# qzwlecr/p1

Measured on AMD Instinct MI355X. Metric: SHA-256 nonce-hashes/sec (GH/s), higher is better.
Workload: dtype u32

## Files before the change

### p1_amd/__init__.py

```python
from ._lib import (
    P1HipError,
    lib_path,
    load,
    init,
    init_devices,
    scan,
    scan_batch,
    batch_layout,
    get_batch_stats,
    hash,
    reduce_pairs,
    plan_shards,
    set_profiling,
    get_stats,
    get_device_stats,
    reset_stats,
    device_count,
    device_info,
    comm_info,
    abi_version,
    ABI_VERSION,
    test_knobs,
    shutdown,
    version,
    codeobj_bytes,
    codeobj_sha256,
    batch_codeobj_sha256,
)
from .sharding import shard_range, combine_keys
```

### p1_amd/_lib.py

```python
import ctypes
import os

_HERE = os.path.dirname(os.path.abspath(__file__))
_LIB = None

U64 = ctypes.c_uint64


class P1HipError(RuntimeError):
    def __init__(self, rc, msg):
        super().__init__(f"p1hip rc={rc}: {msg}")
        self.rc = rc


class Stats(ctypes.Structure):
    _fields_ = [
        ("scans", U64),
        ("fast_launches", U64),
        ("fast_nonces", U64),
        ("fast_alg_ops", U64),
        ("generic_launches", U64),
        ("generic_nonces", U64),
        ("scan_wall_ms", ctypes.c_double),
        ("scan_launches", U64),
# ... 45 lines not shown
        ("launches", U64),
        ("tiles", U64),
        ("nonces", U64),
        ("wall_ms", ctypes.c_double),
    ]

    def as_dict(self):
        return {k: getattr(self, k) for k, _ in self._fields_}


class DeviceInfo(ctypes.Structure):
    _fields_ = [
        ("ordinal", ctypes.c_int32),
        ("cu_count", ctypes.c_int32),
        ("clock_khz", ctypes.c_int32),
        ("reserved", ctypes.c_int32),
        ("hbm_bytes", U64),
        ("pci_bus_id", ctypes.c_char * 32),
        ("arch", ctypes.c_char * 32),
        ("uuid", ctypes.c_ubyte * 16),
    ]

    def as_dict(self):
        return {"ordinal": self.ordinal, "cu_count": self.cu_count, "clock_khz": self.clock_khz,
                "hbm_bytes": self.hbm_bytes, "pci_bus_id": self.pci_bus_id.decode(errors="replace"),
                "arch": self.arch.decode(errors="replace"), "uuid": bytes(self.uuid).hex()}


def lib_path():
    return os.environ.get("P1HIP_LIB") or os.path.join(_HERE, "libp1hip.so")


SIGNATURES = [
    ("p1hip_init", ctypes.c_int, [ctypes.c_int, ctypes.POINTER(ctypes.c_int)]),
    ("p1hip_init_devices", ctypes.c_int, [ctypes.POINTER(ctypes.c_int), ctypes.c_int]),
    ("p1hip_scan", ctypes.c_int,
     [ctypes.c_char_p, ctypes.c_size_t, U64, U64, ctypes.POINTER(U64), ctypes.POINTER(U64)]),
    ("p1hip_scan_batch", ctypes.c_int, [ctypes.POINTER(Request), ctypes.c_size_t, ctypes.POINTER(Result)]),
    ("p1hip_batch_layout", ctypes.c_int,
     [ctypes.POINTER(Request), ctypes.c_size_t, ctypes.c_int, ctypes.POINTER(ctypes.c_uint32),
      ctypes.POINTER(ctypes.c_int32), ctypes.POINTER(ctypes.c_int32)]),
    ("p1hip_get_batch_stats", ctypes.c_int, [ctypes.POINTER(BatchStats)]),
    ("p1hip_hash", ctypes.c_int, [ctypes.c_char_p, ctypes.c_size_t, U64, ctypes.POINTER(U64)]),
    ("p1hip_plan_shards", ctypes.c_int,
     [ctypes.c_char_p, ctypes.c_size_t, U64, U64, ctypes.c_int, ctypes.POINTER(U64), ctypes.POINTER(U64)]),
    ("p1hip_reduce_pairs", ctypes.c_int,
     [ctypes.POINTER(U64), ctypes.POINTER(U64), ctypes.c_size_t, ctypes.POINTER(U64), ctypes.POINTER(U64)]),
    ("p1hip_set_profiling", ctypes.c_int, [ctypes.c_int]),
    ("p1hip_get_stats", ctypes.c_int, [ctypes.POINTER(Stats)]),
    ("p1hip_reset_stats", None, []),
    ("p1hip_get_device_stats", ctypes.c_int, [ctypes.c_int, ctypes.POINTER(DeviceStats)]),
    ("p1hip_device_count", ctypes.c_int, []),
    ("p1hip_device_info", ctypes.c_int, [ctypes.c_int, ctypes.POINTER(DeviceInfo)]),
    ("p1hip_comm_info", ctypes.c_int, [ctypes.c_int, ctypes.POINTER(ctypes.c_int), ctypes.POINTER(ctypes.c_int)]),
    ("p1hip_abi_version", ctypes.c_int, []),
    ("p1hip_test_knobs", ctypes.c_char_p, []),
    ("p1hip_last_error", ctypes.c_char_p, []),
    ("p1hip_version", ctypes.c_char_p, []),
    ("p1hip_shutdown", None, []),
]


def load(path=None):
    global _LIB
    if _LIB is not None and path is None:
        return _LIB
    p = path or lib_path()
    if not os.path.exists(p):
        raise P1HipError(-100, f"{p} not built (run `make` or __graft_entry__.build())")
    lib = ctypes.CDLL(p)
    for name, res, args in SIGNATURES:
        fn = getattr(lib, name)
        fn.restype = res
        fn.argtypes = args
    if lib.p1hip_abi_version() != ABI_VERSION:
        raise P1HipError(-100, f"{p}: ABI version {lib.p1hip_abi_version()}, this binding reads version "
                               f"{ABI_VERSION} structs (rebuild the library)")
    if path is None:
        _LIB = lib
    return lib


def _check(rc):
    if rc != 0:
        raise P1HipError(rc, load().p1hip_last_error().decode(errors="replace"))


def _bytes(msg):
    if isinstance(msg, str):
        return msg.encode("utf-8")
    return bytes(msg)


def init(want_devices=0):
    got = ctypes.c_int(0)
    _check(load().p1hip_init(int(want_devices), ctypes.byref(got)))
    return got.value


def init_devices(ordinals):
    arr = (ctypes.c_int * len(ordinals))(*ordinals)
    _check(load().p1hip_init_devices(arr, len(ordinals)))


def scan(msg, lower, upper):
    m = _bytes(msg)
    h, n = U64(), U64()
    _check(load().p1hip_scan(m, len(m), int(lower), int(upper), ctypes.byref(h), ctypes.byref(n)))
    return h.value, n.value


def _requests(requests):
    rows = [(_bytes(m), int(lo), int(hi)) for m, lo, hi in requests]
    arr = (Request * max(len(rows), 1))()
    for r, (m, lo, hi) in zip(arr, rows):
        r.msg, r.msg_len, r.lower, r.upper = m, len(m), lo, hi
    return arr, rows


def scan_batch(requests):
    arr, rows = _requests(requests)
    out = (Result * max(len(rows), 1))()
    _check(load().p1hip_scan_batch(arr, len(rows), out))
    return [(out[i].hash, out[i].nonce) for i in range(len(rows))]


def batch_layout(requests, ndev):
    arr, rows = _requests(requests)
    n = len(rows)
    tiles = (ctypes.c_uint32 * max(n, 1))()
    device = (ctypes.c_int32 * max(n, 1))()
    launch = (ctypes.c_int32 * max(n, 1))()
    _check(load().p1hip_batch_layout(arr, n, int(ndev), tiles, device, launch))
    return [{"tiles": tiles[i], "device": device[i], "launch": launch[i]} for i in range(n)]


def get_batch_stats():
    s = BatchStats()
    _check(load().p1hip_get_batch_stats(ctypes.byref(s)))
    return s.as_dict()


def batch_codeobj_sha256(lib=None):
    import hashlib

    lib = lib or load()
    start = ctypes.addressof(ctypes.c_char.in_dll(lib, "p1hip_batch_co"))
    end = ctypes.addressof(ctypes.c_char.in_dll(lib, "p1hip_batch_co_end"))
    if end <= start:
        raise P1HipError(-100, "embedded batch code object is empty")
    return hashlib.sha256(ctypes.string_at(start, end - start)).hexdigest()


def hash(msg, nonce):
    m = _bytes(msg)
    h = U64()
    _check(load().p1hip_hash(m, len(m), int(nonce), ctypes.byref(h)))
    return h.value


def plan_shards(msg, lower, upper, n):
    m = _bytes(msg)
    first, last = (U64 * n)(), (U64 * n)()
    _check(load().p1hip_plan_shards(m, len(m), int(lower), int(upper), int(n), first, last))
    return [(a, b) if a <= b else None for a, b in zip(first, last)]


def reduce_pairs(hashes, nonces):
    n = len(hashes)
    assert n == len(nonces)
    ha = (U64 * max(n, 1))(*hashes)
    na = (U64 * max(n, 1))(*nonces)
    h, o = U64(), U64()
    _check(load().p1hip_reduce_pairs(ha, na, n, ctypes.byref(h), ctypes.byref(o)))
    return h.value, o.value


def set_profiling(on):
    _check(load().p1hip_set_profiling(1 if on else 0))


def get_stats():
    s = Stats()
    _check(load().p1hip_get_stats(ctypes.byref(s)))
    return s.as_dict()


def get_device_stats(index):
    s = DeviceStats()
    _check(load().p1hip_get_device_stats(int(index), ctypes.byref(s)))
    return s.as_dict()


def device_info(index):
    s = DeviceInfo()
    _check(load().p1hip_device_info(int(index), ctypes.byref(s)))
    return s.as_dict()


def comm_info(index):
    n, r = ctypes.c_int(0), ctypes.c_int(-1)
    _check(load().p1hip_comm_info(int(index), ctypes.byref(n), ctypes.byref(r)))
    return n.value, r.value


ABI_VERSION = 6


def abi_version():
    return load().p1hip_abi_version()


def test_knobs():
    raw = load().p1hip_test_knobs().decode()
    return dict(kv.split("=", 1) if "=" in kv else (kv, "?") for kv in raw.split(";") if kv)


def reset_stats():
    load().p1hip_reset_stats()


def device_count():
    return load().p1hip_device_count()


def shutdown():
    load().p1hip_shutdown()


def version():
    return load().p1hip_version().decode()


def codeobj_bytes(lib=None):
    lib = lib or load()
    start = ctypes.addressof(ctypes.c_char.in_dll(lib, "p1hip_kernels_co"))
    end = ctypes.addressof(ctypes.c_char.in_dll(lib, "p1hip_kernels_co_end"))
    if end <= start:
        raise P1HipError(-100, "embedded code object is empty")
    return ctypes.string_at(start, end - start)


def codeobj_sha256(lib=None):
    import hashlib

    return hashlib.sha256(codeobj_bytes(lib)).hexdigest()
```

### p1_amd/csrc/p1hip.hip

```cpp
#include <hip/hip_runtime.h>
#include <rccl/rccl.h>

#include <stdlib.h>
#include <string.h>

#include <algorithm>
#include <atomic>
#include <chrono>
#include <exception>
#include <mutex>
#include <string>
#include <thread>
#include <utility>
#include <vector>

#include "../../include/p1hip.h"
#include "batch_plan.hpp"
#include "planner.hpp"
#include "scan_abi.hpp"
#include "scan_pack.hpp"

extern "C" const unsigned char p1hip_kernels_co[];
extern "C" const unsigned char p1hip_batch_co[];

using namespace p1;

namespace {

thread_local std::string g_err;

int fail(int rc, const std::string& what) {
  g_err = what;
  return rc;
}

template <typename Fn>
int guarded(Fn&& fn) {
  try {
    return fn();
  } catch (const std::exception& ex) {
    return fail(P1HIP_ERR_HIP, std::string("host: ") + ex.what());
  } catch (...) {
    return fail(P1HIP_ERR_HIP, "host: unknown exception");
  }
}

#define HIPCHK(expr)                                                                        \
  do {                                                                                      \
    hipError_t e_ = (expr);                                                                 \
    if (e_ != hipSuccess)                                                                   \
      return fail(P1HIP_ERR_HIP, std::string(#expr) + ": " + hipGetErrorString(e_));       \
  } while (0)

#define NCCLCHK(expr)                                                                       \
  do {                                                                                      \
    ncclResult_t r_ = (expr);                                                               \
    if (r_ != ncclSuccess)                                                                  \
      return fail(P1HIP_ERR_RCCL, std::string(#expr) + ": " + ncclGetErrorString(r_));      \
  } while (0)

constexpr size_t kMaxKwTabs = 8;
constexpr uint64_t kMaxKwTabBytes = 8ull << 30;
constexpr uint64_t kMaxScanSpan = 1ull << 40;

enum KnobKind { kValue, kZeroDef, kFlag };
enum KnobWhen { kPerScan, kPerBatch, kAtInit };
enum KnobId {
  kSmallMaxNoncesKnob, kMaxLaunchBlocksKnob, kMaxScanSpanKnob, kKwtabMaxBytesKnob, kNoRcclKnob, kForceRcclKnob,
  kMinFastThreadsKnob, kTestFailDeviceKnob, kNoTableKnob, kNoSplitKnob, kScanGridKnob, kBatchMaxNoncesKnob,
  kBatchMaxTilesKnob, kKnobCount
};
struct Knob {
  const char* name;
  uint64_t def, max;
  KnobKind kind;
  KnobWhen when;
  const char* what;
};
const Knob kKnobs[] = {
    {"P1HIP_SMALL_MAX_NONCES", kSmallMaxNonces, kSmallMaxNonces, kValue, kPerScan,
     "shares of at most this many nonces take the one-launch small path; 0 turns it off, so small parity ranges "
     "run the fast kernel variants"},
    {"P1HIP_MAX_LAUNCH_BLOCKS", kMaxLaunchBlocks, kMaxLaunchBlocks, kZeroDef, kPerScan,
     "workgroups per k_scan launch, so GPU tests run the multi-launch path on small ranges; a larger piece gets "
     "a launch of its own (at most kMaxFastThreads / kBlock = 2^18 workgroups, far below HIP's grid limit)"},
    {"P1HIP_MAX_SCAN_SPAN", kMaxScanSpan, ~0ull, kZeroDef, kPerScan, "nonces per piece of a device's share"},
    {"P1HIP_KWTAB_MAX_BYTES", kMaxKwTabBytes, ~0ull, kValue, kPerScan,
     "MODE 5 table cap; a larger table re-plans the share without MODE 5"},
    {"P1HIP_NO_RCCL", 0, 1, kFlag, kAtInit,
     "combine the per-device results through the host, so the multi-device path (threads, sharding, combine) "
     "runs with the same GPU listed twice on a 1-GPU box"},
    {"P1HIP_FORCE_RCCL", 0, 1, kFlag, kAtInit, "a communicator even for one device"},
    {"P1HIP_MIN_FAST_THREADS", kMinFastThreads, ~0ull, kValue, kAtInit,
     "planner occupancy floor; 1 keeps k = 3 on small ranges so every k = 3 variant runs on the GPU"},
    {"P1HIP_TEST_FAIL_DEVICE", ~0ull, ~0ull, kValue, kAtInit,
     "device index whose scan phase reports a failure (the multi-device error path); default -1: none"},
    {"P1HIP_NO_TABLE", 0, 1, kFlag, kAtInit,
     "no MODE 5: layouts whose tail block 1 holds only lo digits run the digit-update variants (A/B, and a "
     "second kernel path to cross-check MODE 5)"},
    {"P1HIP_NO_SPLIT", 0, 1, kFlag, kAtInit,
     "straddling lo digits use mode 2 instead of the split modes (A/B builds with -DP1_NV2_PLAIN)"},
    {"P1HIP_SCAN_GRID", 0, kMaxLaunchBlocks, kZeroDef, kPerScan,
     "k_scan's grid instead of the device's workgroup slots (the default, 0); at or above a launch's tile count "
     "every workgroup runs one tile and the queue hands out none (the round-5 dispatch, same code object)"},
    {"P1HIP_BATCH_MAX_NONCES", kBatchMaxNonces, kBatchMaxNonces, kValue, kPerBatch,
     "requests of at most this many nonces are coalesced by p1hip_scan_batch; 0 runs every request "
     "individually; independent of P1HIP_SMALL_MAX_NONCES"},
    {"P1HIP_BATCH_MAX_TILES", kBatchMaxTiles, kBatchMaxTiles, kZeroDef, kPerBatch,
     "tiles per launch pair, so GPU tests run several launch pairs on small batches (batch_layout raises it to "
     "the largest single request's tile count)"},
};
static_assert(sizeof kKnobs / sizeof kKnobs[0] == kKnobCount, "one row per KnobId, in its order");

bool test_knobs_on() {
  const char* m = getenv("P1HIP_TEST_KNOBS");
  return m && m[0] == '1' && m[1] == 0;
}

const char* test_knob(const char* name) {
  if (!test_knobs_on()) return nullptr;
  const char* v = getenv(name);
  return v && *v ? v : nullptr;
}

uint64_t knob(KnobId id) {
  const Knob& K = kKnobs[id];
  const char* v = test_knob(K.name);
  if (!v) return K.def;
  if (K.kind == kFlag) return v[0] == '1';
  const uint64_t n = strtoull(v, nullptr, 10);
  if (n == 0 && K.kind == kZeroDef) return K.def;
  return n < K.max ? n : K.max;
}

template <typename T, bool kPinned>
struct Buf {
  T* p = nullptr;
  size_t cap = 0;

  Buf() = default;
  Buf(const Buf&) = delete;
  Buf(Buf&& o) noexcept : p(std::exchange(o.p, nullptr)), cap(std::exchange(o.cap, 0)) {}
  Buf& operator=(Buf&& o) noexcept {
    if (this != &o) {
      (void)release();
      p = std::exchange(o.p, nullptr);
      cap = std::exchange(o.cap, 0);
    }
    return *this;
  }
  ~Buf() { (void)release(); }

  hipError_t release() {
    hipError_t e = hipSuccess;
    if (p) e = kPinned ? hipHostFree(p) : hipFree(p);
    p = nullptr;
    cap = 0;
    return e;
  }
  hipError_t reserve(size_t need, size_t floor, size_t extra = 0) {
    if (need <= cap) return hipSuccess;
    hipError_t e = release();
    if (e != hipSuccess) return e;
    size_t n = floor;
    while (n < need) n <<= 1;
    const size_t bytes = (n + extra) * sizeof(T);
    e = kPinned ? hipHostMalloc(&p, bytes, hipHostMallocDefault) : hipMalloc(&p, bytes);
    if (e != hipSuccess) p = nullptr;
    else cap = n;
    return e;
  }
};
template <typename T> using DevBuf = Buf<T, false>;
template <typename T> using PinnedBuf = Buf<T, true>;

struct Dev {
  int ordinal = -1;
  hipStream_t stream = nullptr;
  DevBuf<Key> d_part;
  DevBuf<Key> d_res;
  DevBuf<Key> d_gather;
  PinnedBuf<Key> h_res;
  DevBuf<Segment> d_seg;
  PinnedBuf<Segment> h_seg;
  ncclComm_t comm = nullptr;
  hipModule_t mod = nullptr;
  hipFunction_t f_scan = nullptr, f_reduce = nullptr, f_pairs = nullptr, f_small = nullptr, f_kwtable = nullptr;
  DevBuf<Key> d_small_part;
  DevBuf<uint32_t> d_ticket;
  DevBuf<uint32_t> d_scan_ticket;
  uint32_t scan_grid = 0;
  bool small_used = false;
  hipModule_t bmod = nullptr;
  hipFunction_t f_bscan = nullptr, f_breduce = nullptr;
  DevBuf<BatchSeg> d_bseg;
  PinnedBuf<BatchSeg> h_bseg;
  DevBuf<uint32_t> d_btile0;
  PinnedBuf<uint32_t> h_btile0;
  DevBuf<Key> d_bout;
  PinnedBuf<Key> h_bout;
  DevBuf<Key> d_bpart;
  std::vector<hipEvent_t> evs;
  struct KwTab {
    uint32_t w[16];
    int k;
    uint32_t* dptr;
    uint64_t used_in;
  };
  std::vector<KwTab> kwtabs;
  uint64_t range_id = 0;
  ScanCounters ctr;
  uint64_t replans = 0;
  p1hip_device_stats_t acc{};
};

struct Runtime {
  std::mutex mu;
  std::vector<Dev> devs;
  bool profiling = false;
  bool use_rccl = true;
  bool rccl_one = false;
  uint64_t min_fast_threads = kMinFastThreads;
  bool split = true;
  bool tabulate = true;
  int fail_device = -1;
  p1hip_stats_t stats{};
  p1hip_batch_stats_t bstats{};
};

Runtime& rt() {
  static Runtime* r = new Runtime();
  return *r;
}

int device_count(int* count) {
  *count = 0;
  if (hipGetDeviceCount(count) != hipSuccess || *count <= 0)
    return fail(P1HIP_ERR_NO_DEVICE, "no HIP device visible");
  return P1HIP_OK;
}

template <typename... Args>
hipError_t launch(hipFunction_t f, uint32_t blocks, uint32_t threads, hipStream_t st, Args... args) {
  void* params[] = {(void*)&args...};
  return hipModuleLaunchKernel(f, blocks, 1, 1, threads, 1, 1, 0, st, params, nullptr);
}

int ev_record(Dev& d, size_t& nev) {
  if (d.evs.size() <= nev) {
    hipEvent_t e;
    HIPCHK(hipEventCreate(&e));
    d.evs.push_back(e);
  }
  HIPCHK(hipEventRecord(d.evs[nev], d.stream));
  ++nev;
  return P1HIP_OK;
}

int ev_sum(Dev& d, size_t nev) {
  if (!nev) return P1HIP_OK;
  HIPCHK(hipEventSynchronize(d.evs[nev - 1]));
  for (size_t i = 0; i + 1 < nev; i += 2) {
    float ms = 0.f;
    HIPCHK(hipEventElapsedTime(&ms, d.evs[i], d.evs[i + 1]));
    d.ctr.scan_ms += ms;
  }
  return P1HIP_OK;
}

Key finish_key(Key k) {
  if (k.h == ~0ull) k.n = 0;
  return k;
}

void add_counters(p1hip_stats_t& s, const ScanCounters& c) {
  s.fast_launches += c.fast_launches;
  s.fast_nonces += c.fast_nonces;
  s.fast_alg_ops += c.fast_ops;
  s.generic_launches += c.gen_launches;
  s.generic_nonces += c.gen_nonces;
  s.scan_launches += c.scan_launches;
  s.scan_nonces += c.scan_nonces;
  s.scan_alg_ops += c.scan_ops;
  s.scan_kernel_ms += c.scan_ms;
}

void add_counters(p1hip_device_stats_t& a, const ScanCounters& c) {
  a.scans++;
  a.scan_launches += c.scan_launches;
  a.scan_nonces += c.scan_nonces;
  a.scan_alg_ops += c.scan_ops;
  a.scan_kernel_ms += c.scan_ms;
}

int dev_release(Dev& d) {
  if (d.ordinal < 0) return 0;
  (void)hipSetDevice(d.ordinal);
  if (d.stream) (void)hipStreamSynchronize(d.stream);
  for (hipEvent_t e : d.evs) (void)hipEventDestroy(e);
  for (Dev::KwTab& t : d.kwtabs) (void)hipFree(t.dptr);
  if (d.comm) ncclCommDestroy(d.comm);
  if (d.stream) (void)hipStreamDestroy(d.stream);
  if (d.mod) (void)hipModuleUnload(d.mod);
  if (d.bmod) (void)hipModuleUnload(d.bmod);
  d = Dev();
  return 0;
}

void shutdown_locked(Runtime& R) {
  for (Dev& d : R.devs) dev_release(d);
  R.devs.clear();
}

int init_devs(Runtime& R, const std::vector<int>& ords) {
  int count = 0;
  if (int rc = device_count(&count)) return rc;
  const int nd = (int)ords.size();
  std::vector<int> cus(ords.size());
  for (int i = 0; i < nd; ++i) {
    const int o = ords[i];
    if (o < 0 || o >= count) return fail(P1HIP_ERR_NO_DEVICE, "device ordinal out of range: " + std::to_string(o));
    hipDeviceProp_t prop;
    HIPCHK(hipGetDeviceProperties(&prop, o));
    if (std::string(prop.gcnArchName).rfind("gfx950", 0) != 0)
      return fail(P1HIP_ERR_NO_DEVICE, std::string("device is not gfx950: ") + prop.gcnArchName);
    cus[i] = prop.multiProcessorCount;
  }
  R.devs.resize(ords.size());
  for (int i = 0; i < nd; ++i) {
    Dev& d = R.devs[i];
    d.ordinal = ords[i];
    HIPCHK(hipSetDevice(d.ordinal));
    HIPCHK(hipStreamCreateWithFlags(&d.stream, hipStreamNonBlocking));
    HIPCHK(hipModuleLoadData(&d.mod, p1hip_kernels_co));
    HIPCHK(hipModuleGetFunction(&d.f_scan, d.mod, "k_scan"));
    HIPCHK(hipModuleGetFunction(&d.f_reduce, d.mod, "k_reduce"));
    HIPCHK(hipModuleGetFunction(&d.f_pairs, d.mod, "k_pairs"));
    HIPCHK(hipModuleGetFunction(&d.f_small, d.mod, "k_scan_small"));
    HIPCHK(hipModuleGetFunction(&d.f_kwtable, d.mod, "k_kwtable"));
    HIPCHK(hipModuleLoadData(&d.bmod, p1hip_batch_co));
    HIPCHK(hipModuleGetFunction(&d.f_bscan, d.bmod, "k_batch_scan"));
    HIPCHK(hipModuleGetFunction(&d.f_breduce, d.bmod, "k_batch_reduce"));
    HIPCHK(d.d_small_part.reserve(kSmallMaxBlocks, kSmallMaxBlocks));
    HIPCHK(d.d_ticket.reserve(1, 1));
    HIPCHK(d.d_scan_ticket.reserve(2, 2));
    HIPCHK(hipMemsetAsync(d.d_ticket.p, 0, sizeof(uint32_t), d.stream));
    HIPCHK(hipMemsetAsync(d.d_scan_ticket.p, 0, 2 * sizeof(uint32_t), d.stream));
    int per_cu = 0;
    HIPCHK(hipModuleOccupancyMaxActiveBlocksPerMultiprocessor(&per_cu, d.f_scan, kBlock, 0));
    if (per_cu < 1 || cus[i] < 1)
      return fail(P1HIP_ERR_HIP, "k_scan occupancy: " + std::to_string(per_cu) + " blocks per CU");
    d.scan_grid = (uint32_t)per_cu * (uint32_t)cus[i];
    HIPCHK(hipStreamSynchronize(d.stream));
    HIPCHK(d.d_res.reserve(1, 1));
    HIPCHK(d.d_gather.reserve((size_t)nd, (size_t)nd));
    HIPCHK(d.h_res.reserve((size_t)nd, (size_t)nd));
  }
  R.use_rccl = !knob(kNoRcclKnob);
  R.rccl_one = knob(kForceRcclKnob) && R.use_rccl;
  R.min_fast_threads = knob(kMinFastThreadsKnob);
  R.split = !knob(kNoSplitKnob);
  R.tabulate = !knob(kNoTableKnob);
  R.fail_device = (int)(int64_t)knob(kTestFailDeviceKnob);
  if ((nd > 1 || R.rccl_one) && R.use_rccl) {
    std::vector<ncclComm_t> comms(nd);
    NCCLCHK(ncclCommInitAll(comms.data(), nd, ords.data()));
    for (int i = 0; i < nd; ++i) R.devs[i].comm = comms[i];
  }
  return P1HIP_OK;
}

int init_locked(Runtime& R, const std::vector<int>& ords) {
  if (!R.devs.empty()) {
    bool same = R.devs.size() == ords.size();
    for (size_t i = 0; same && i < ords.size(); ++i) same = R.devs[i].ordinal == ords[i];
    if (same) return P1HIP_OK;
    shutdown_locked(R);
  }
  const int rc = init_devs(R, ords);
  if (rc != P1HIP_OK) {
    const std::string keep = g_err;
    shutdown_locked(R);
    g_err = keep;
  }
  return rc;
}

int ensure_init(Runtime& R) {
  if (!R.devs.empty()) return P1HIP_OK;
  int count = 0;
  if (int rc = device_count(&count)) return rc;
  std::vector<int> ords;
  for (int i = 0; i < count; ++i) ords.push_back(i);
  return init_locked(R, ords);
}

int run_small(Dev& d, const uint8_t* msg, size_t len, uint64_t lo, uint64_t hi, bool to_host, bool profiling) {
  HIPCHK(hipSetDevice(d.ordinal));
  d.ctr = {};
  Plan plan;
  std::string err = make_plan(msg, len, lo, hi, plan, false);
  if (!err.empty()) return fail(P1HIP_ERR_ARGS, "planner: " + err);
  SmallArgs a;
  err = fill_small(plan, a, d.ctr);
  if (!err.empty()) return fail(P1HIP_ERR_ARGS, err);
  a.part = d.d_small_part.p;
  a.ticket = d.d_ticket.p;
  a.out_dev = d.d_res.p;
  a.out_host = to_host ? d.h_res.p : nullptr;
  int rc;
  size_t nev = 0;
  if (profiling && (rc = ev_record(d, nev))) return rc;
  HIPCHK(launch(d.f_small, a.nblocks, kBlock, d.stream, a));
  if (profiling && (rc = ev_record(d, nev))) return rc;
  return ev_sum(d, nev);
}

constexpr int kNoTable = 1;

int kwtable_for(Dev& d, const Launch& L, uint64_t* dptr) {
  for (size_t i = 0; i < d.kwtabs.size(); ++i) {
    Dev::KwTab t = d.kwtabs[i];
    if (t.k == L.tabk && memcmp(t.w, L.tabw, sizeof t.w) == 0) {
      t.used_in = d.range_id;
      d.kwtabs.erase(d.kwtabs.begin() + (long)i);
      d.kwtabs.push_back(t);
      *dptr = (uint64_t)(uintptr_t)t.dptr;
      return P1HIP_OK;
    }
  }
  const size_t need = (size_t)pow10u(L.tabk) * 64u * sizeof(uint32_t);
  const size_t cap = (size_t)knob(kKwtabMaxBytesKnob);
  if (need > cap) return kNoTable;
  for (;;) {
    size_t held = 0;
    for (const Dev::KwTab& t : d.kwtabs) held += (size_t)pow10u(t.k) * 64u * sizeof(uint32_t);
    if (d.kwtabs.empty() || (d.kwtabs.size() < kMaxKwTabs && held + need <= cap)) break;
    size_t v = 0;
    while (v < d.kwtabs.size() && d.kwtabs[v].used_in == d.range_id) ++v;
    if (v == d.kwtabs.size()) return kNoTable;
    HIPCHK(hipFree(d.kwtabs[v].dptr));
    d.kwtabs.erase(d.kwtabs.begin() + (long)v);
  }
  Dev::KwTab t;
  memcpy(t.w, L.tabw, sizeof t.w);
  t.k = L.tabk;
  t.dptr = nullptr;
  t.used_in = d.range_id;
  const uint32_t rows = (uint32_t)pow10u(L.tabk);
  const hipError_t me = hipMalloc(&t.dptr, (size_t)rows * 64u * sizeof(uint32_t));
  if (me == hipErrorOutOfMemory) {
    (void)hipGetLastError();
    return kNoTable;
  }
  HIPCHK(me);
  KwTableArgs a;
  memset(&a, 0, sizeof a);
  memcpy(a.tabw, L.tabw, sizeof a.tabw);
  a.k = (uint32_t)L.tabk;
  a.qv = (uint32_t)(L.Y.q - 64);
  a.rows = rows;
  a.out = t.dptr;
  const hipError_t e = launch(d.f_kwtable, (rows + kBlock - 1) / kBlock, kBlock, d.stream, a);
  if (e != hipSuccess) {
    (void)hipFree(t.dptr);
    return fail(P1HIP_ERR_HIP, std::string("k_kwtable launch: ") + hipGetErrorString(e));
  }
  d.kwtabs.push_back(t);
  *dptr = (uint64_t)(uintptr_t)t.dptr;
  return P1HIP_OK;
}

uint32_t scan_grid_for(const Dev& d, uint32_t tiles) {
  const uint64_t g = knob(kScanGridKnob);
  return std::min(tiles, g > 0 ? (uint32_t)g : d.scan_grid);
}

int run_range(Dev& d, const uint8_t* msg, size_t len, uint64_t lo, uint64_t hi, bool profiling,
              uint64_t min_fast_threads, bool split, bool tabulate) {
  HIPCHK(hipSetDevice(d.ordinal));
  d.range_id++;
  d.ctr = {};
  Plan plan;
  std::vector<uint64_t> tabptr;
  for (;;) {
    std::string err = make_plan(msg, len, lo, hi, plan, true, min_fast_threads, split, tabulate);
    if (!err.empty()) return fail(P1HIP_ERR_ARGS, "planner: " + err);
    tabptr.assign(plan.launches.size(), 0);
    bool replan = false;
    for (size_t i = 0; i < plan.launches.size() && !replan; ++i) {
      const Launch& L = plan.launches[i];
      if (!L.fast || (L.mode != 5 && L.mode != 7)) continue;
      const int rt = kwtable_for(d, L, &tabptr[i]);
      if (rt == kNoTable) replan = true;
      else if (rt != P1HIP_OK) return rt;
    }
    if (!replan) break;
    tabulate = false;
    d.replans++;
    plan = Plan();
  }
  const ScanPack P = pack_scan(plan, knob(kMaxLaunchBlocksKnob));
  HIPCHK(d.d_part.reserve(P.total_blocks, 1));
  HIPCHK(d.d_seg.reserve(P.batches.size() * kMaxSegs, 4 * kMaxSegs));
  HIPCHK(d.h_seg.reserve(P.batches.size() * kMaxSegs, 4 * kMaxSegs));
  int rc;
  size_t nev = 0;
  uint32_t part_off = 0;
  for (size_t bi = 0; bi < P.batches.size(); ++bi) {
    const ScanBatch& B = P.batches[bi];
    Segment* hs = d.h_seg.p + bi * kMaxSegs;
    Segment* ds = d.d_seg.p + bi * kMaxSegs;
    const std::string err = fill_segments(plan, P, B, tabptr.data(), hs, d.ctr);
    if (!err.empty()) return fail(P1HIP_ERR_ARGS, err);
    HIPCHK(hipMemcpyAsync(ds, hs, B.count * sizeof(Segment), hipMemcpyHostToDevice, d.stream));
    if (profiling && (rc = ev_record(d, nev))) return rc;
#ifdef P1_STATIC_GRID
    HIPCHK(launch(d.f_scan, B.blocks, kBlock, d.stream, (const Segment*)ds, (uint32_t)B.count,
                  (Key*)(d.d_part.p + part_off)));
#else
    HIPCHK(launch(d.f_scan, scan_grid_for(d, B.blocks), kBlock, d.stream, (const Segment*)ds,
                  (uint32_t)B.count, (Key*)(d.d_part.p + part_off), (uint32_t)B.blocks, d.d_scan_ticket.p));
#endif
    if (profiling && (rc = ev_record(d, nev))) return rc;
    part_off += B.blocks;
  }
  HIPCHK(launch(d.f_reduce, 1, kReduceThreads, d.stream, (const Key*)d.d_part.p, P.total_blocks, d.d_res.p));
  return ev_sum(d, nev);
}

int run_share(Dev& d, const uint8_t* msg, size_t len, uint64_t lo, uint64_t hi, const Runtime& R) {
  const uint64_t span = knob(kMaxScanSpanKnob);
  if (hi - lo < span)
    return run_range(d, msg, len, lo, hi, R.profiling, R.min_fast_threads, R.split, R.tabulate);
  Key best = {~0ull, ~0ull};
  ScanCounters sum;
  for (uint64_t a = lo;;) {
    const uint64_t b = hi - a < span ? hi : a + (span - 1);
    int r = run_range(d, msg, len, a, b, R.profiling, R.min_fast_threads, R.split, R.tabulate);
    if (r != P1HIP_OK) return r;
    Key k;
    HIPCHK(hipMemcpyAsync(&k, d.d_res.p, sizeof(Key), hipMemcpyDeviceToHost, d.stream));
    HIPCHK(hipStreamSynchronize(d.stream));
    if (key_lt(k, best)) best = k;
    sum += d.ctr;
    if (b == hi) break;
    a = b + 1;
  }
  d.ctr = sum;
  HIPCHK(hipMemcpyAsync(d.d_res.p, &best, sizeof(Key), hipMemcpyHostToDevice, d.stream));
  HIPCHK(hipStreamSynchronize(d.stream));
  return P1HIP_OK;
}

int scan_held(Runtime& R, const uint8_t* msg, size_t msg_len, uint64_t lower, uint64_t upper, uint64_t* out_hash,
              uint64_t* out_nonce) {
  const auto t0 = std::chrono::steady_clock::now();
  int rc = ensure_init(R);
  if (rc) return rc;
  Key res = {~0ull, 0};
  if (lower <= upper) {
    const size_t nd = R.devs.size();
    std::vector<uint64_t> slo(nd), shi(nd);
    std::vector<char> active(nd, 0);
    plan_shards(msg, msg_len, lower, upper, (int)nd, slo.data(), shi.data());
    for (size_t i = 0; i < nd; ++i) active[i] = slo[i] <= shi[i];
    std::vector<int> rcs(nd, 0);
    std::vector<std::string> errs(nd);
    auto run_threads = [&](auto&& fn) {
      if (nd == 1) {
        fn(0);
      } else {
        std::atomic<int> go{0};
        std::vector<std::thread> th;
        try {
          for (size_t i = 0; i < nd; ++i)
            th.emplace_back([&, i]() {
              while (go.load(std::memory_order_acquire) == 0) std::this_thread::yield();
              if (go.load(std::memory_order_acquire) == 1) fn(i);
            });
        } catch (...) {
          go.store(-1, std::memory_order_release);
          for (auto& t : th) t.join();
          throw;
        }
        go.store(1, std::memory_order_release);
        for (auto& t : th) t.join();
      }
    };
    auto run_phase = [&](double p1hip_device_stats_t::*ms, auto&& body) {
      run_threads([&](size_t i) {
        Dev& d = R.devs[i];
        const auto p0 = std::chrono::steady_clock::now();
        int r;
        try {
          r = body(i, d);
        } catch (const std::exception& ex) {
          try {
            r = fail(P1HIP_ERR_HIP, std::string("host: ") + ex.what());
          } catch (...) {
            r = P1HIP_ERR_HIP;
          }
        } catch (...) {
          r = P1HIP_ERR_HIP;
        }
        d.acc.*ms += std::chrono::duration<double, std::milli>(std::chrono::steady_clock::now() - p0).count();
        rcs[i] = r;
        if (r) {
          try {
            errs[i] = g_err;
          } catch (...) {
          }
        }
      });
      for (size_t i = 0; i < nd; ++i)
        if (rcs[i]) return fail(rcs[i], "device " + std::to_string(R.devs[i].ordinal) + ": " + errs[i]);
      return (int)P1HIP_OK;
    };
    const bool coll = (nd > 1 || R.rccl_one) && R.use_rccl;
    const uint64_t small_max = knob(kSmallMaxNoncesKnob);
    rc = run_phase(&p1hip_device_stats_t::phase1_ms, [&](size_t i, Dev& d) -> int {
      d.ctr = {};
      d.replans = 0;
      d.small_used = false;
      d.acc.shard_first = slo[i];
      d.acc.shard_last = shi[i];
      d.acc.active = active[i];
      int r = P1HIP_OK;
      if ((int)i == R.fail_device) {
        r = fail(P1HIP_ERR_HIP, "injected failure (P1HIP_TEST_FAIL_DEVICE)");
      } else if (active[i] && shi[i] - slo[i] < small_max) {
        d.small_used = true;
        r = run_small(d, msg, msg_len, slo[i], shi[i], !coll && nd == 1, R.profiling);
      } else if (active[i]) {
        r = run_share(d, msg, msg_len, slo[i], shi[i], R);
      } else {
        if (hipSetDevice(d.ordinal) != hipSuccess) r = fail(P1HIP_ERR_HIP, "hipSetDevice");
        if (!r && hipMemsetAsync(d.d_res.p, 0xFF, sizeof(Key), d.stream) != hipSuccess)
          r = fail(P1HIP_ERR_HIP, "hipMemsetAsync(identity)");
      }
      if (!r && !coll && nd > 1) {
        if (hipMemcpyAsync(R.devs[0].h_res.p + i, d.d_res.p, sizeof(Key), hipMemcpyDeviceToHost, d.stream) !=
            hipSuccess)
          r = fail(P1HIP_ERR_HIP, "hipMemcpyAsync(result)");
      } else if (!r && !coll && !(active[i] && d.small_used)) {
        if (hipMemcpyAsync(d.h_res.p, d.d_res.p, sizeof(Key), hipMemcpyDeviceToHost, d.stream) != hipSuccess)
          r = fail(P1HIP_ERR_HIP, "hipMemcpyAsync(result)");
      }
      if (!r && hipStreamSynchronize(d.stream) != hipSuccess) r = fail(P1HIP_ERR_HIP, "hipStreamSynchronize");
      return r;
    });
    if (rc != P1HIP_OK) return rc;
    if (coll) {
      rc = run_phase(&p1hip_device_stats_t::gather_ms, [&](size_t i, Dev& d) -> int {
        if (hipSetDevice(d.ordinal) != hipSuccess) return fail(P1HIP_ERR_HIP, "hipSetDevice");
        ncclResult_t nr = ncclAllGather(d.d_res.p, d.d_gather.p, 2, ncclUint64, d.comm, d.stream);
        if (nr != ncclSuccess) return fail(P1HIP_ERR_RCCL, std::string("ncclAllGather: ") + ncclGetErrorString(nr));
        if (i == 0 &&
            hipMemcpyAsync(d.h_res.p, d.d_gather.p, sizeof(Key) * nd, hipMemcpyDeviceToHost, d.stream) != hipSuccess)
          return fail(P1HIP_ERR_HIP, "hipMemcpyAsync(gathered)");
        if (hipStreamSynchronize(d.stream) != hipSuccess) return fail(P1HIP_ERR_HIP, "hipStreamSynchronize");
        return P1HIP_OK;
      });
      if (rc != P1HIP_OK) return rc;
    }
    Key b = {~0ull, ~0ull};
    for (size_t i = 0; i < nd; ++i) b = key_lt(R.devs[0].h_res.p[i], b) ? R.devs[0].h_res.p[i] : b;
    res = finish_key(b);
    for (Dev& d : R.devs) {
      add_counters(R.stats, d.ctr);
      add_counters(d.acc, d.ctr);
      if (d.small_used && d.ctr.scan_launches) R.stats.small_scans++;
      R.stats.table_replans += d.replans;
    }
// ... 381 lines not shown
```

### p1_amd/csrc/scan_pack.hpp

```cpp
#pragma once
#include <string.h>

#include <algorithm>
#include <string>
#include <vector>

#include "planner.hpp"
#include "scan_abi.hpp"

namespace p1 {

constexpr uint32_t kMaxSegs = 64;
constexpr uint32_t kMaxLaunchBlocks = 1u << 22;

inline bool has_variant(int fv, int mode, bool trail) {
#define P1_CASE(FV, MODE, TR) \
  if (fv == FV && mode == MODE && trail == TR) return true;
#include "fast_variants.inc"
#undef P1_CASE
  return false;
}

struct ScanCounters {
  uint64_t fast_launches = 0, fast_nonces = 0, fast_ops = 0, gen_launches = 0, gen_nonces = 0;
  uint64_t scan_launches = 0, scan_nonces = 0, scan_ops = 0;
  double scan_ms = 0.0;
  ScanCounters& operator+=(const ScanCounters& o) {
    fast_launches += o.fast_launches; fast_nonces += o.fast_nonces; fast_ops += o.fast_ops;
    gen_launches += o.gen_launches; gen_nonces += o.gen_nonces;
    scan_launches += o.scan_launches; scan_nonces += o.scan_nonces; scan_ops += o.scan_ops;
    scan_ms += o.scan_ms;
    return *this;
  }
};

struct ScanBatch {
  size_t first, count;
  uint32_t blocks;
};

struct ScanPack {
  std::vector<size_t> order;
  std::vector<ScanBatch> batches;
  uint32_t total_blocks = 0;
};

inline ScanPack pack_scan(const Plan& plan, uint64_t max_blocks, uint32_t max_segs = kMaxSegs) {
  ScanPack P;
  P.order.resize(plan.launches.size());
  for (size_t i = 0; i < P.order.size(); ++i) P.order[i] = i;
  auto weight = [&](size_t i) -> uint64_t {
    const Launch& L = plan.launches[i];
    return L.fast ? (uint64_t)(L.fa.kpow / L.fa.nsub) * (uint64_t)L.btail : (uint64_t)L.btail - 1;
  };
  std::stable_sort(P.order.begin(), P.order.end(), [&](size_t a, size_t b) { return weight(a) > weight(b); });
  uint64_t all_blocks = 0;
  for (const Launch& L : plan.launches) all_blocks += L.blocks;
  const uint64_t nlaunch = (all_blocks + max_blocks - 1) / max_blocks;
  const uint64_t target = nlaunch > 1 ? (all_blocks + nlaunch - 1) / nlaunch : max_blocks;
  for (size_t r = 0; r < P.order.size(); ++r) {
    const Launch& L = plan.launches[P.order[r]];
    const uint64_t cur = P.batches.empty() ? 0 : P.batches.back().blocks;
    if (P.batches.empty() || P.batches.back().count == max_segs || cur + (uint64_t)L.blocks > max_blocks ||
        (cur > 0 && cur + L.blocks / 2 > target && P.batches.size() < nlaunch))
      P.batches.push_back({r, 0, 0});
    P.batches.back().count++;
    P.batches.back().blocks += L.blocks;
    P.total_blocks += L.blocks;
  }
  return P;
}

inline std::string fill_segments(const Plan& plan, const ScanPack& P, const ScanBatch& B, const uint64_t* tabptr,
                                 Segment* segs, ScanCounters& c) {
  uint32_t block0 = 0;
  for (size_t j = 0; j < B.count; ++j) {
    const size_t i = P.order[B.first + j];
    const Launch& L = plan.launches[i];
    Segment& S = segs[j];
    memset(&S, 0, sizeof S);
    S.block0 = block0;
    block0 += L.blocks;
    if (L.fast) {
      if (!has_variant(L.fv, L.mode, L.trail)) return "no fast kernel variant";
      S.kind = variant_id(L.fv, L.mode, L.trail);
      S.fa = L.fa;
      if (L.mode == 5 || L.mode == 7) S.fa.kwtab = tabptr[i];
      c.fast_launches++;
      c.fast_nonces += L.nonces;
      c.fast_ops += L.nonces * kAlgOpsPerCompression * (uint64_t)L.btail;
    } else {
      S.kind = kGenericKind;
      S.ga = L.ga;
      c.gen_launches++;
      c.gen_nonces += L.nonces;
    }
    c.scan_nonces += L.nonces;
    c.scan_ops += L.nonces * kAlgOpsPerCompression * (uint64_t)L.btail;
  }
  c.scan_launches++;
  return "";
}

inline std::string fill_small(const Plan& plan, SmallArgs& a, ScanCounters& c) {
  if (plan.launches.size() > kSmallMaxSegs || plan.total_blocks > kSmallMaxBlocks)
    return "internal: small plan exceeds its argument block";
  memset(&a, 0, sizeof a);
  uint32_t block0 = 0;
  for (size_t i = 0; i < plan.launches.size(); ++i) {
    const Launch& L = plan.launches[i];
    a.ga[i] = L.ga;
    a.block0[i] = block0;
    block0 += L.blocks;
    c.gen_launches++;
    c.gen_nonces += L.nonces;
    c.scan_ops += L.nonces * kAlgOpsPerCompression * (uint64_t)L.btail;
  }
  a.nseg = (uint32_t)plan.launches.size();
  a.nblocks = block0;
  c.scan_launches++;
  c.scan_nonces += plan.total_nonces;
  return "";
}

}
```

Measured before the change: 51.51.

## Add dedicated table-scan kernel for MODE 5 pieces with scalar row prefetch

Adds a separate code object with k_scan_tab, a persistent-grid kernel that handles MODE 5 table pieces with k >= 5 lo digits. It loads each 64-word table row as four 16-dword scalar-memory quarters, prefetches the next row while computing rounds, and uses sched barriers to keep the load/compute order. The packer now sorts and batches table pieces separately so they launch on their own kernel with an occupancy-derived grid and ticket. This costs an extra module, an ELF kernarg-size check, and separate launches per kernel type.

```diff
diff --git a/p1_amd/__init__.py b/p1_amd/__init__.py
--- a/p1_amd/__init__.py
+++ b/p1_amd/__init__.py
@@ -26,5 +26,7 @@
     codeobj_bytes,
     codeobj_sha256,
     batch_codeobj_sha256,
+    tab_codeobj_bytes,
+    tab_codeobj_sha256,
 )
 from .sharding import shard_range, combine_keys
diff --git a/p1_amd/_lib.py b/p1_amd/_lib.py
--- a/p1_amd/_lib.py
+++ b/p1_amd/_lib.py
@@ -221,6 +221,21 @@
     return hashlib.sha256(ctypes.string_at(start, end - start)).hexdigest()
 
 
+def tab_codeobj_bytes(lib=None):
+    lib = lib or load()
+    start = ctypes.addressof(ctypes.c_char.in_dll(lib, "p1hip_tab_co"))
+    end = ctypes.addressof(ctypes.c_char.in_dll(lib, "p1hip_tab_co_end"))
+    if end <= start:
+        raise P1HipError(-100, "embedded table-kernel code object is empty")
+    return ctypes.string_at(start, end - start)
+
+
+def tab_codeobj_sha256(lib=None):
+    import hashlib
+
+    return hashlib.sha256(tab_codeobj_bytes(lib)).hexdigest()
+
+
 def hash(msg, nonce):
     m = _bytes(msg)
     h = U64()
diff --git a/p1_amd/csrc/p1hip.hip b/p1_amd/csrc/p1hip.hip
--- a/p1_amd/csrc/p1hip.hip
+++ b/p1_amd/csrc/p1hip.hip
@@ -1,6 +1,7 @@
 #include <hip/hip_runtime.h>
 #include <rccl/rccl.h>
 
+#include <elf.h>
 #include <stdlib.h>
 #include <string.h>
 
@@ -22,6 +23,8 @@
 
 extern "C" const unsigned char p1hip_kernels_co[];
 extern "C" const unsigned char p1hip_batch_co[];
+extern "C" const unsigned char p1hip_tab_co[];
+extern "C" const unsigned char p1hip_tab_co_end[];
 
 using namespace p1;
 
@@ -68,7 +71,7 @@
 enum KnobId {
   kSmallMaxNoncesKnob, kMaxLaunchBlocksKnob, kMaxScanSpanKnob, kKwtabMaxBytesKnob, kNoRcclKnob, kForceRcclKnob,
   kMinFastThreadsKnob, kTestFailDeviceKnob, kNoTableKnob, kNoSplitKnob, kScanGridKnob, kBatchMaxNoncesKnob,
-  kBatchMaxTilesKnob, kKnobCount
+  kBatchMaxTilesKnob, kTabKernelKnob, kKnobCount
 };
 struct Knob {
   const char* name;
@@ -109,6 +112,9 @@
     {"P1HIP_BATCH_MAX_TILES", kBatchMaxTiles, kBatchMaxTiles, kZeroDef, kPerBatch,
      "tiles per launch pair, so GPU tests run several launch pairs on small batches (batch_layout raises it to "
      "the largest single request's tile count)"},
+    {"P1HIP_TAB_KERNEL", 1, 1, kValue, kPerScan,
+     "0 keeps MODE 5 pieces with k >= 5 lo digits on k_scan instead of k_scan_tab (A/B, and a second kernel path "
+     "to cross-check the table kernel)"},
 };
 static_assert(sizeof kKnobs / sizeof kKnobs[0] == kKnobCount, "one row per KnobId, in its order");
 
@@ -191,6 +197,10 @@
   DevBuf<uint32_t> d_scan_ticket;
   uint32_t scan_grid = 0;
   bool small_used = false;
+  hipModule_t tmod = nullptr;
+  hipFunction_t f_tab = nullptr;
+  DevBuf<uint32_t> d_tab_ticket;
+  uint32_t tab_grid = 0;
   hipModule_t bmod = nullptr;
   hipFunction_t f_bscan = nullptr, f_breduce = nullptr;
   DevBuf<BatchSeg> d_bseg;
@@ -303,6 +313,7 @@
   if (d.stream) (void)hipStreamDestroy(d.stream);
   if (d.mod) (void)hipModuleUnload(d.mod);
   if (d.bmod) (void)hipModuleUnload(d.bmod);
+  if (d.tmod) (void)hipModuleUnload(d.tmod);
   d = Dev();
   return 0;
 }
@@ -310,6 +321,38 @@
 void shutdown_locked(Runtime& R) {
   for (Dev& d : R.devs) dev_release(d);
   R.devs.clear();
+}
+
+uint32_t kernarg_bytes(const unsigned char* elf, const unsigned char* end, const std::string& name) {
+  const size_t n = (size_t)(end - elf);
+  Elf64_Ehdr eh;
+  if (n < sizeof eh) return 0;
+  memcpy(&eh, elf, sizeof eh);
+  if (memcmp(eh.e_ident, ELFMAG, SELFMAG) != 0 || eh.e_ident[EI_CLASS] != ELFCLASS64 ||
+      eh.e_shentsize != sizeof(Elf64_Shdr) || eh.e_shoff > n || (n - eh.e_shoff) / sizeof(Elf64_Shdr) < eh.e_shnum)
+    return 0;
+  std::vector<Elf64_Shdr> sh(eh.e_shnum);
+  if (!sh.empty()) memcpy(sh.data(), elf + eh.e_shoff, sh.size() * sizeof(Elf64_Shdr));
+  auto inside = [&](const Elf64_Shdr& s) { return s.sh_type != SHT_NOBITS && s.sh_offset <= n && s.sh_size <= n - s.sh_offset; };
+  const std::string want = name + ".kd";
+  for (const Elf64_Shdr& st : sh) {
+    if ((st.sh_type != SHT_SYMTAB && st.sh_type != SHT_DYNSYM) || !inside(st) || st.sh_link >= sh.size()) continue;
+    const Elf64_Shdr& str = sh[st.sh_link];
+    if (!inside(str)) continue;
+    for (size_t i = 0; i < st.sh_size / sizeof(Elf64_Sym); ++i) {
+      Elf64_Sym sym;
+      memcpy(&sym, elf + st.sh_offset + i * sizeof sym, sizeof sym);
+      if (sym.st_name >= str.sh_size || sym.st_shndx >= sh.size()) continue;
+      const char* nm = (const char*)elf + str.sh_offset + sym.st_name;
+      if (strnlen(nm, str.sh_size - sym.st_name) != want.size() || memcmp(nm, want.data(), want.size()) != 0) continue;
+      const Elf64_Shdr& sec = sh[sym.st_shndx];
+      if (!inside(sec) || sym.st_value < sec.sh_addr || sym.st_value - sec.sh_addr + 12 > sec.sh_size) return 0;
+      uint32_t v;
+      memcpy(&v, elf + sec.sh_offset + (sym.st_value - sec.sh_addr) + 8, sizeof v);
+      return v;
+    }
+  }
+  return 0;
 }
 
 int init_devs(Runtime& R, const std::vector<int>& ords) {
@@ -341,16 +384,29 @@
     HIPCHK(hipModuleLoadData(&d.bmod, p1hip_batch_co));
     HIPCHK(hipModuleGetFunction(&d.f_bscan, d.bmod, "k_batch_scan"));
     HIPCHK(hipModuleGetFunction(&d.f_breduce, d.bmod, "k_batch_reduce"));
+    HIPCHK(hipModuleLoadData(&d.tmod, p1hip_tab_co));
+    HIPCHK(hipModuleGetFunction(&d.f_tab, d.tmod, "k_scan_tab"));
+    const uint32_t tab_args = kernarg_bytes(p1hip_tab_co, p1hip_tab_co_end, "k_scan_tab");
+    if (tab_args != kScanKernargBytes + kHiddenKernargBytes)
+      return fail(P1HIP_ERR_HIP, "k_scan_tab takes " + std::to_string(tab_args) + " argument bytes, the library passes " +
+                                     std::to_string(kScanKernargBytes + kHiddenKernargBytes));
     HIPCHK(d.d_small_part.reserve(kSmallMaxBlocks, kSmallMaxBlocks));
     HIPCHK(d.d_ticket.reserve(1, 1));
     HIPCHK(d.d_scan_ticket.reserve(2, 2));
+    HIPCHK(d.d_tab_ticket.reserve(2, 2));
     HIPCHK(hipMemsetAsync(d.d_ticket.p, 0, sizeof(uint32_t), d.stream));
     HIPCHK(hipMemsetAsync(d.d_scan_ticket.p, 0, 2 * sizeof(uint32_t), d.stream));
+    HIPCHK(hipMemsetAsync(d.d_tab_ticket.p, 0, 2 * sizeof(uint32_t), d.stream));
     int per_cu = 0;
     HIPCHK(hipModuleOccupancyMaxActiveBlocksPerMultiprocessor(&per_cu, d.f_scan, kBlock, 0));
     if (per_cu < 1 || cus[i] < 1)
       return fail(P1HIP_ERR_HIP, "k_scan occupancy: " + std::to_string(per_cu) + " blocks per CU");
     d.scan_grid = (uint32_t)per_cu * (uint32_t)cus[i];
+    per_cu = 0;
+    HIPCHK(hipModuleOccupancyMaxActiveBlocksPerMultiprocessor(&per_cu, d.f_tab, kBlock, 0));
+    if (per_cu < 1)
+      return fail(P1HIP_ERR_HIP, "k_scan_tab occupancy: " + std::to_string(per_cu) + " blocks per CU");
+    d.tab_grid = (uint32_t)per_cu * (uint32_t)cus[i];
     HIPCHK(hipStreamSynchronize(d.stream));
     HIPCHK(d.d_res.reserve(1, 1));
     HIPCHK(d.d_gather.reserve((size_t)nd, (size_t)nd));
@@ -471,9 +527,9 @@
   return P1HIP_OK;
 }
 
-uint32_t scan_grid_for(const Dev& d, uint32_t tiles) {
+uint32_t scan_grid_for(const Dev& d, uint32_t tiles, ScanKernel kernel) {
   const uint64_t g = knob(kScanGridKnob);
-  return std::min(tiles, g > 0 ? (uint32_t)g : d.scan_grid);
+  return std::min(tiles, g > 0 ? (uint32_t)g : kernel == kKernelTab ? d.tab_grid : d.scan_grid);
 }
 
 int run_range(Dev& d, const uint8_t* msg, size_t len, uint64_t lo, uint64_t hi, bool profiling,
@@ -500,7 +556,7 @@
     d.replans++;
     plan = Plan();
   }
-  const ScanPack P = pack_scan(plan, knob(kMaxLaunchBlocksKnob));
+  const ScanPack P = pack_scan(plan, knob(kMaxLaunchBlocksKnob), kMaxSegs, knob(kTabKernelKnob) != 0);
   HIPCHK(d.d_part.reserve(P.total_blocks, 1));
   HIPCHK(d.d_seg.reserve(P.batches.size() * kMaxSegs, 4 * kMaxSegs));
   HIPCHK(d.h_seg.reserve(P.batches.size() * kMaxSegs, 4 * kMaxSegs));
@@ -514,12 +570,21 @@
     const std::string err = fill_segments(plan, P, B, tabptr.data(), hs, d.ctr);
     if (!err.empty()) return fail(P1HIP_ERR_ARGS, err);
     HIPCHK(hipMemcpyAsync(ds, hs, B.count * sizeof(Segment), hipMemcpyHostToDevice, d.stream));
+    if (B.kernel == kKernelTab) {
+      HIPCHK(hipMemsetAsync(d.d_tab_ticket.p, 0, 2 * sizeof(uint32_t), d.stream));
+      if (profiling && (rc = ev_record(d, nev))) return rc;
+      HIPCHK(launch(d.f_tab, scan_grid_for(d, B.blocks, kKernelTab), kBlock, d.stream, (const Segment*)ds,
+                    (uint32_t)B.count, (Key*)(d.d_part.p + part_off), (uint32_t)B.blocks, d.d_tab_ticket.p));
+      if (profiling && (rc = ev_record(d, nev))) return rc;
+      part_off += B.blocks;
+      continue;
+    }
     if (profiling && (rc = ev_record(d, nev))) return rc;
 #ifdef P1_STATIC_GRID
     HIPCHK(launch(d.f_scan, B.blocks, kBlock, d.stream, (const Segment*)ds, (uint32_t)B.count,
                   (Key*)(d.d_part.p + part_off)));
 #else
-    HIPCHK(launch(d.f_scan, scan_grid_for(d, B.blocks), kBlock, d.stream, (const Segment*)ds,
+    HIPCHK(launch(d.f_scan, scan_grid_for(d, B.blocks, kKernelScan), kBlock, d.stream, (const Segment*)ds,
                   (uint32_t)B.count, (Key*)(d.d_part.p + part_off), (uint32_t)B.blocks, d.d_scan_ticket.p));
 #endif
     if (profiling && (rc = ev_record(d, nev))) return rc;
diff --git a/p1_amd/csrc/p1hip_tab_blob.S b/p1_amd/csrc/p1hip_tab_blob.S
--- /dev/null
+++ b/p1_amd/csrc/p1hip_tab_blob.S
@@ -0,0 +1,13 @@
+/* Embeds the gfx950 code object built from p1hip_tab_kernels.hip (Makefile:
+   build/p1hip_tab.hsaco) into libp1hip.so, after the scan and batch objects
+   (the scan object stays the first AMDGPU ELF in the library)
+   loads it with hipModuleLoadData on every device it initialises. */
+    .section .rodata
+    .balign 4096
+    .globl p1hip_tab_co
+    .type p1hip_tab_co, @object
+p1hip_tab_co:
+    .incbin P1HIP_TAB_CO
+    .globl p1hip_tab_co_end
+p1hip_tab_co_end:
+    .section .note.GNU-stack,"",@progbits
diff --git a/p1_amd/csrc/p1hip_tab_kernels.hip b/p1_amd/csrc/p1hip_tab_kernels.hip
--- /dev/null
+++ b/p1_amd/csrc/p1hip_tab_kernels.hip
@@ -0,0 +1,33 @@
+#include <hip/hip_runtime.h>
+
+#include "scan_abi.hpp"
+#include "scan_tab.hpp"
+
+using namespace p1;
+
+#include "argmin_dev.hpp"
+
+extern "C" __global__ __launch_bounds__(kBlock, 4) void k_scan_tab(const Segment* __restrict__ segs, uint32_t nseg,
+                                                                   Key* __restrict__ part, uint32_t ntiles,
+                                                                   uint32_t* __restrict__ ticket) {
+  __shared__ uint32_t s_next;
+  uint32_t b = blockIdx.x;
+  for (;;) {
+    uint32_t si = 0;
+    while (si + 1 < nseg && segs[si + 1].block0 <= b) ++si;
+    const Segment& S = segs[si];
+    Key k = {~0ull, ~0ull};
+    if (S.kind == variant_id(0, 5, false)) k = tab_thread_uniform(S.fa, (b - S.block0) * kBlock + threadIdx.x);
+    block_min_store<kBlock>(k, part + b);
+    if (threadIdx.x == 0)
+      s_next = gridDim.x + __hip_atomic_fetch_add(&ticket[0], 1u, __ATOMIC_RELAXED, __HIP_MEMORY_SCOPE_AGENT);
+    __syncthreads();
+    b = (uint32_t)__builtin_amdgcn_readfirstlane((int)s_next);
+    if (b >= ntiles) break;
+  }
+  if (threadIdx.x == 0 &&
+      __hip_atomic_fetch_add(&ticket[1], 1u, __ATOMIC_RELAXED, __HIP_MEMORY_SCOPE_AGENT) == gridDim.x - 1) {
+    __hip_atomic_store(&ticket[0], 0u, __ATOMIC_RELAXED, __HIP_MEMORY_SCOPE_AGENT);
+    __hip_atomic_store(&ticket[1], 0u, __ATOMIC_RELAXED, __HIP_MEMORY_SCOPE_AGENT);
+  }
+}
diff --git a/p1_amd/csrc/scan_pack.hpp b/p1_amd/csrc/scan_pack.hpp
--- a/p1_amd/csrc/scan_pack.hpp
+++ b/p1_amd/csrc/scan_pack.hpp
@@ -34,9 +34,19 @@
   }
 };
 
+enum ScanKernel : uint32_t { kKernelScan = 0, kKernelTab = 1 };
+constexpr int kTabMinK = 5;
+constexpr uint32_t kScanKernargBytes = 40;
+constexpr uint32_t kHiddenKernargBytes = 256;
+
+inline ScanKernel kernel_of(const Launch& L, bool use_tab) {
+  return use_tab && L.fast && L.mode == 5 && L.tabk >= kTabMinK ? kKernelTab : kKernelScan;
+}
+
 struct ScanBatch {
   size_t first, count;
   uint32_t blocks;
+  ScanKernel kernel;
 };
 
 struct ScanPack {
@@ -45,7 +55,7 @@
   uint32_t total_blocks = 0;
 };
 
-inline ScanPack pack_scan(const Plan& plan, uint64_t max_blocks, uint32_t max_segs = kMaxSegs) {
+inline ScanPack pack_scan(const Plan& plan, uint64_t max_blocks, uint32_t max_segs = kMaxSegs, bool use_tab = true) {
   ScanPack P;
   P.order.resize(plan.launches.size());
   for (size_t i = 0; i < P.order.size(); ++i) P.order[i] = i;
@@ -53,20 +63,30 @@
     const Launch& L = plan.launches[i];
     return L.fast ? (uint64_t)(L.fa.kpow / L.fa.nsub) * (uint64_t)L.btail : (uint64_t)L.btail - 1;
   };
-  std::stable_sort(P.order.begin(), P.order.end(), [&](size_t a, size_t b) { return weight(a) > weight(b); });
-  uint64_t all_blocks = 0;
-  for (const Launch& L : plan.launches) all_blocks += L.blocks;
-  const uint64_t nlaunch = (all_blocks + max_blocks - 1) / max_blocks;
-  const uint64_t target = nlaunch > 1 ? (all_blocks + nlaunch - 1) / nlaunch : max_blocks;
-  for (size_t r = 0; r < P.order.size(); ++r) {
-    const Launch& L = plan.launches[P.order[r]];
-    const uint64_t cur = P.batches.empty() ? 0 : P.batches.back().blocks;
-    if (P.batches.empty() || P.batches.back().count == max_segs || cur + (uint64_t)L.blocks > max_blocks ||
-        (cur > 0 && cur + L.blocks / 2 > target && P.batches.size() < nlaunch))
-      P.batches.push_back({r, 0, 0});
-    P.batches.back().count++;
-    P.batches.back().blocks += L.blocks;
-    P.total_blocks += L.blocks;
+  auto kern = [&](size_t i) { return kernel_of(plan.launches[i], use_tab); };
+  std::stable_sort(P.order.begin(), P.order.end(), [&](size_t a, size_t b) {
+    if (kern(a) != kern(b)) return kern(a) == kKernelTab;
+    return weight(a) > weight(b);
+  });
+  size_t r = 0;
+  for (const ScanKernel K : {kKernelTab, kKernelScan}) {
+    uint64_t all_blocks = 0;
+    for (size_t i = 0; i < plan.launches.size(); ++i)
+      if (kern(i) == K) all_blocks += plan.launches[i].blocks;
+    const uint64_t nlaunch = (all_blocks + max_blocks - 1) / max_blocks;
+    const uint64_t target = nlaunch > 1 ? (all_blocks + nlaunch - 1) / nlaunch : max_blocks;
+    const size_t batch0 = P.batches.size();
+    for (; r < P.order.size() && kern(P.order[r]) == K; ++r) {
+      const Launch& L = plan.launches[P.order[r]];
+      const bool none = P.batches.size() == batch0;
+      const uint64_t cur = none ? 0 : P.batches.back().blocks;
+      if (none || P.batches.back().count == max_segs || cur + (uint64_t)L.blocks > max_blocks ||
+          (cur > 0 && cur + L.blocks / 2 > target && P.batches.size() - batch0 < nlaunch))
+        P.batches.push_back({r, 0, 0, K});
+      P.batches.back().count++;
+      P.batches.back().blocks += L.blocks;
+      P.total_blocks += L.blocks;
+    }
   }
   return P;
 }
diff --git a/p1_amd/csrc/scan_tab.hpp b/p1_amd/csrc/scan_tab.hpp
--- /dev/null
+++ b/p1_amd/csrc/scan_tab.hpp
@@ -0,0 +1,80 @@
+#pragma once
+#include <string.h>
+
+#include "scan_core.hpp"
+
+namespace p1 {
+
+typedef uint32_t RowQuarter __attribute__((ext_vector_type(16)));
+
+P1_HD RowQuarter ld_quarter(const uint32_t* p) {
+#if defined(__HIP_DEVICE_COMPILE__)
+  return *(const __attribute__((address_space(4))) RowQuarter*)p;
+#else
+  RowQuarter q;
+  memcpy(&q, p, sizeof q);
+  return q;
+#endif
+}
+
+P1_HD void sched_fence() {
+#if defined(__HIP_DEVICE_COMPILE__)
+  __builtin_amdgcn_sched_barrier(0);
+#endif
+}
+
+template <int T0, int T1>
+P1_HD void quarter_rounds(State& s, const RowQuarter& q) {
+#pragma unroll
+  for (int t = T0; t < T1; ++t) sha_round(s, q[t & 15]);
+}
+
+P1_HD uint32_t tab_prefetch_row(uint32_t c, uint32_t c_last) { return c < c_last ? c + 1u : c_last; }
+
+P1_HD Key tab_thread_uniform(const FastArgs& A, uint32_t tid) {
+  const uint32_t wv = tid >> 6, lane = tid & 63u;
+  const uint32_t sub = wave_uniform(wv % A.nsub);
+  const uint32_t hid = (wv / A.nsub) * 64u + lane;
+  const uint32_t per = A.kpow / A.nsub;
+  const uint32_t c0 = sub * per;
+  const uint32_t c_last = c0 + per - 1u;
+  FastSetup S;
+  fast_setup(A, hid, S);
+  State s0, s1;
+#pragma unroll
+  for (int i = 0; i < 8; ++i) s0.v[i] = S.cv[i];
+  round_half<0>(s0, s1);
+  const uint32_t* tab = (const uint32_t*)(uintptr_t)A.kwtab;
+  uint64_t best = ~0ull;
+  uint32_t bestc = 0;
+  RowQuarter q0 = ld_quarter(tab + (size_t)c0 * 64u);
+  for (uint32_t c = c0; c <= c_last; ++c) {
+    const uint32_t* row = tab + (size_t)c * 64u;
+    State s = s1;
+    s.v[0] = add2(s.v[0], q0[0]);
+    s.v[4] = add2(s.v[4], q0[0]);
+    sched_fence();
+    const RowQuarter q1 = ld_quarter(row + 16);
+    const RowQuarter q2 = ld_quarter(row + 32);
+    const RowQuarter q3 = ld_quarter(row + 48);
+    sched_fence();
+    quarter_rounds<1, 16>(s, q0);
+    quarter_rounds<16, 17>(s, q1);
+    sched_fence();
+    q0 = ld_quarter(tab + (size_t)tab_prefetch_row(c, c_last) * 64u);
+    sched_fence();
+    quarter_rounds<17, 32>(s, q1);
+    quarter_rounds<32, 48>(s, q2);
+    quarter_rounds<48, 64>(s, q3);
+    const uint64_t h = ((uint64_t)(S.cv[0] + s.v[0]) << 32) | (uint64_t)(S.cv[1] + s.v[1]);
+    const bool lt = h < best;
+    best = lt ? h : best;
+    bestc = lt ? c : bestc;
+  }
+  Key k;
+  k.h = S.valid ? best : ~0ull;
+  k.n = S.valid ? S.hi * (uint64_t)A.kpow + bestc : ~0ull;
+  return k;
+}
+
+}
```

After: 51.50, median of 2. No clear change (-0.0%).
